# canyagmur/XPoint

Hardware: AMD Instinct MI355X
Metric: image-pairs/sec (detect+describe+match) 480x640 optical-thermal (higher is better)
Workload: dtype f32 (dense layers: f32 operands as 2 fp16 terms (operand error <= 2^-23, dropped cross term <= 2^-22: per product <= 2^-21 worst case, ~2^-25 typical), 3 fp16-MFMA partial products, f32 accumulate — GEMMs, implicit-GEMM convolutions and the fused block kernels alike; the deep-stage scan's dt project

## Files before the change

xpoint_amd/csrc/ss2d_chunked.hip:

```cpp
#include <string>

#include "ss2d_core.h"

namespace {

template <int R, typename UT = float>
__device__ __forceinline__ void stage_chunk(const SS2DParams& p, int T, int b, int pair, int chunk0, int* s_pix, int* s_off, float* s_x) {
    const int L = p.H * p.W;
    const int npx = p.cpb * T;
    const int tsh = 31 - __builtin_clz(T);
    for (int i = threadIdx.x; i < npx; i += blockDim.x) {
        int cl = i >> tsh, ii = i - (cl << tsh);
        int chunk = chunk0 + cl;
        const int px = (chunk < p.nc) ? pixel_of((chunk << tsh) + ii, L, p.H, p.W, pair == 1) : -1;
        s_pix[i] = px;
        s_off[i] = px >= 0 ? px * p.C : -1;
    }
    __syncthreads();
    constexpr int XW = 2 * (R + 2);
    constexpr int XD = 2 * XW;
    const UT* xsrc = reinterpret_cast<const UT*>(p.xdbl) + (int64_t)b * L * XD + pair * XW;
    for (int i = threadIdx.x; i < npx * XW; i += blockDim.x) {
        int pi = i / XW, e = i - pi * XW;
        int px = s_pix[pi];
        s_x[i] = (px >= 0) ? (float)xsrc[(int64_t)px * XD + e] : 0.f;
    }
    __syncthreads();
}

#define XP_PASS1_LOAD_U4(uv)                                                                                            \
    int px[4];                                                                                                          \
    _Pragma("unroll") for (int k = 0; k < 4; ++k) {                                                                     \
        px[k] = s_off[cl * p.T + i0 + k];                                                                               \
        const float t = (XP_SS2D_DBG & 8) ? 1.f : (float)ub[(FULL || px[k] >= 0) ? px[k] : 0];                          \
        uv[k] = (FULL || px[k] >= 0) ? t : 0.f;                                                                         \
    }

template <int R, bool FULL, bool AMP = false, typename UT = float>
__global__ __launch_bounds__(768) void ss2d_pass1(SS2DParams p) {
    constexpr float WL2E = AMP ? 1.f : XP_L2E;
    extern __shared__ __align__(16) char smem[];
    const int npx = p.cpb * p.T;
    int* s_pix = reinterpret_cast<int*>(smem);
    int* s_off = s_pix + npx;
    float* s_x = reinterpret_cast<float*>(smem + sizeof(int) * 2 * npx);
    constexpr int XW = 2 * (R + 2);
    const int b = blockIdx.y, pair = blockIdx.z, chunk0 = blockIdx.x * p.cpb;
    stage_chunk<R, UT>(p, p.T, b, pair, chunk0, s_pix, s_off, s_x);
    const int cl = threadIdx.x / p.C, c = threadIdx.x - cl * p.C;
    const int chunk = chunk0 + cl;
    if (chunk >= p.nc) return;
    const int L = p.H * p.W;
    const UT* ub = reinterpret_cast<const UT*>(p.u) + (int64_t)b * L * p.C + c;
    float P0 = 1.f, S0 = 0.f, Q1 = 1.f, S1 = 0.f;
    if constexpr (R < 16) {
        float w0[R], w1[R];
#pragma unroll
        for (int r = 0; r < R; ++r) {
            w0[r] = WL2E * p.wdt[((int64_t)(pair * 2 + 0) * R + r) * p.C + c];
            w1[r] = WL2E * p.wdt[((int64_t)(pair * 2 + 1) * R + r) * p.C + c];
        }
        const float b0 = WL2E * p.dtb[(pair * 2 + 0) * p.C + c], b1 = WL2E * p.dtb[(pair * 2 + 1) * p.C + c];
        const float A0 = XP_L2E * p.A[(pair * 2 + 0) * p.C + c], A1 = XP_L2E * p.A[(pair * 2 + 1) * p.C + c];
        for (int i0 = 0; i0 < p.T; i0 += 4) {
            float uv[4];
            XP_PASS1_LOAD_U4(uv)
#pragma unroll
            for (int k = 0; k < 4; ++k) {
                const float* xr = s_x + (cl * p.T + i0 + k) * XW;
                float a, bb, cv;
                step_vals<R, AMP>(xr, w0, b0, A0, uv[k], a, bb, cv);
                S0 = a * S0 + bb; P0 *= a;
                step_vals<R, AMP>(xr + (R + 2), w1, b1, A1, uv[k], a, bb, cv);
                S1 = fmaf(Q1, bb, S1); Q1 *= a;
            }
        }
    } else {
#pragma unroll 1
    for (int route = 0; route < 2; ++route) {
        float w[R];
#pragma unroll
        for (int r = 0; r < R; ++r) w[r] = WL2E * p.wdt[((int64_t)(pair * 2 + route) * R + r) * p.C + c];
        const float bias = WL2E * p.dtb[(pair * 2 + route) * p.C + c], Av = XP_L2E * p.A[(pair * 2 + route) * p.C + c];
        float Pr = 1.f, Sr = 0.f;
        for (int i0 = 0; i0 < p.T; i0 += 4) {
            float uv[4];
            XP_PASS1_LOAD_U4(uv)
#pragma unroll
            for (int k = 0; k < 4; ++k) {
                const float* xr = s_x + (cl * p.T + i0 + k) * XW + route * (R + 2);
                float a, bb, cv;
                step_vals<R, AMP>(xr, w, bias, Av, uv[k], a, bb, cv);
                if (route == 0) Sr = a * Sr + bb;
                else Sr = fmaf(Pr, bb, Sr);
                Pr *= a;
            }
        }
        if (route == 0) { P0 = Pr; S0 = Sr; } else { Q1 = Pr; S1 = Sr; }
    }
    }
    const int64_t o = ((((int64_t)b * 2 + pair) * p.nc + chunk) * 2) * p.C + c;
    p.wsP[o] = P0; p.wsS[o] = S0;
    p.wsP[o + p.C] = Q1; p.wsS[o + p.C] = S1;
}

#ifndef XP_SS2D_P2G
#define XP_SS2D_P2G 16
#endif
constexpr int P2_G = XP_SS2D_P2G;
__global__ __launch_bounds__(64 * P2_G) void ss2d_pass2(SS2DParams p) {
    __shared__ float s_P[P2_G][64], s_S[P2_G][64];
    const int lane = threadIdx.x, g = threadIdx.y;
    const int c = blockIdx.x * 64 + lane;
    const int bp = blockIdx.y >> 1, dir = blockIdx.y & 1;
    const bool ok = c < p.C;
    const int per = (p.nc + P2_G - 1) / P2_G;
    const int j0 = g * per, j1 = min(p.nc, j0 + per);
    auto off = [&](int jj) -> int64_t {
        const int j = dir ? (p.nc - 1 - jj) : jj;
        return (((int64_t)bp * p.nc + j) * 2 + dir) * p.C + c;
    };
    float P = 1.f, S = 0.f;
    if (ok) {
        int jj = j0;
        for (; jj + 4 <= j1; jj += 4) {
            float Pv[4], Sv[4];
#pragma unroll
            for (int k = 0; k < 4; ++k) { const int64_t o = off(jj + k); Pv[k] = p.wsP[o]; Sv[k] = p.wsS[o]; }
#pragma unroll
            for (int k = 0; k < 4; ++k) { S = fmaf(Pv[k], S, Sv[k]); P *= Pv[k]; }
        }
        for (; jj < j1; ++jj) { const int64_t o = off(jj); const float Pj = p.wsP[o], Sj = p.wsS[o]; S = fmaf(Pj, S, Sj); P *= Pj; }
    }
    s_P[g][lane] = P; s_S[g][lane] = S;
    __syncthreads();
    float h = 0.f;
    for (int gg = 0; gg < g; ++gg) h = fmaf(s_P[gg][lane], h, s_S[gg][lane]);
    if (!ok) return;
    int jj = j0;
    for (; jj + 4 <= j1; jj += 4) {
        float Pv[4], Sv[4];
        int64_t ov[4];
#pragma unroll
        for (int k = 0; k < 4; ++k) { ov[k] = off(jj + k); Pv[k] = p.wsP[ov[k]]; Sv[k] = p.wsS[ov[k]]; }
#pragma unroll
        for (int k = 0; k < 4; ++k) { p.wsS[ov[k]] = h; h = fmaf(Pv[k], h, Sv[k]); }
    }
    for (; jj < j1; ++jj) { const int64_t o = off(jj); const float Pj = p.wsP[o], Sj = p.wsS[o]; p.wsS[o] = h; h = fmaf(Pj, h, Sj); }
}

template <int R, bool COLPAIR, bool FULL, int T, bool AMP = false, typename UT = float>
__global__ __launch_bounds__(768) void ss2d_pass3(SS2DParams p) {
    constexpr float WL2E = AMP ? 1.f : XP_L2E;
    extern __shared__ __align__(16) char smem[];
    const int npx = p.cpb * T;
    int* s_pix = reinterpret_cast<int*>(smem);
    int* s_off = s_pix + npx;
    float* s_x = reinterpret_cast<float*>(smem + sizeof(int) * 2 * npx);
    constexpr int XW = 2 * (R + 2);
    float* s_y = s_x + npx * XW;
    const int SY = p.C + 8;
    const int pair = COLPAIR ? 1 : 0;
    const int b = blockIdx.y, chunk0 = blockIdx.x * p.cpb;
    stage_chunk<R, UT>(p, T, b, pair, chunk0, s_pix, s_off, s_x);
    const int cl = threadIdx.x / p.C, c = threadIdx.x - cl * p.C;
    const int chunk = chunk0 + cl;
    const int L = p.H * p.W;
    if (chunk < p.nc) {
        const int* so = s_off + cl * T;
        const float* sx = s_x + cl * T * XW;
        float* sy = s_y + cl * T * SY + c;
        const UT* ub = reinterpret_cast<const UT*>(p.u) + (int64_t)b * L * p.C + c;
        const float* prev = COLPAIR ? (p.ya + (int64_t)b * L * p.C + c) : nullptr;
        float* dst = COLPAIR ? nullptr : (p.ya + (int64_t)b * L * p.C + c);
        float w0[R];
#pragma unroll
        for (int r = 0; r < R; ++r) w0[r] = WL2E * p.wdt[((int64_t)(pair * 2 + 0) * R + r) * p.C + c];
        const float b0 = WL2E * p.dtb[(pair * 2 + 0) * p.C + c];
        const float A0 = XP_L2E * p.A[(pair * 2 + 0) * p.C + c];
        const float D0 = p.Dp[(pair * 2 + 0) * p.C + c];
        const int64_t o = ((((int64_t)b * 2 + pair) * p.nc + chunk) * 2) * p.C + c;
        float h = p.wsS[o];
        float uv[T], pv[COLPAIR ? T : 1];
#pragma unroll
        for (int i = 0; i < T; ++i) {
            const int off = so[i];
            const float t = (XP_SS2D_DBG & 8) ? 1.f : (float)ub[(FULL || off >= 0) ? off : 0];
            uv[i] = (FULL || off >= 0) ? t : 0.f;
            if ((i & 7) == 7) __builtin_amdgcn_sched_barrier(0);
        }
        if (COLPAIR) {
#pragma unroll
            for (int i = T - 1; i >= 0; --i) {
                const int off = so[i];
                pv[i] = (XP_SS2D_DBG & 2) ? 0.f : prev[(FULL || off >= 0) ? off : 0];
                if ((i & 7) == 0) __builtin_amdgcn_sched_barrier(0);
            }
        }
        __builtin_amdgcn_sched_barrier(0);
#pragma unroll
        for (int i0 = 0; i0 < T; i0 += 4) {
#pragma unroll
            for (int i = i0; i < i0 + 4; ++i) {
                float a, bb, cv;
                float ui = uv[i];
                asm("" : "+v"(ui));
                step_vals<R, AMP>(sx + i * XW, w0, b0, A0, ui, a, bb, cv);
                h = a * h + bb;
                sy[i * SY] = cv * h + D0 * ui;
            }
            __builtin_amdgcn_sched_barrier(0);
        }
        asm volatile("" ::: "memory");
        float w1[R];
#pragma unroll
        for (int r = 0; r < R; ++r) w1[r] = WL2E * p.wdt[((int64_t)(pair * 2 + 1) * R + r) * p.C + c];
        const float b1 = WL2E * p.dtb[(pair * 2 + 1) * p.C + c];
        const float A1 = XP_L2E * p.A[(pair * 2 + 1) * p.C + c];
        const float D1 = p.Dp[(pair * 2 + 1) * p.C + c];
        h = p.wsS[o + p.C];
        __builtin_amdgcn_sched_barrier(0);
#pragma unroll
        for (int i0 = T - 4; i0 >= 0; i0 -= 4) {
#pragma unroll
            for (int i = i0 + 3; i >= i0; --i) {
                float a, bb, cv;
                float ui = uv[i];
                asm("" : "+v"(ui));
                step_vals<R, AMP>(sx + i * XW + (R + 2), w1, b1, A1, ui, a, bb, cv);
                h = a * h + bb;
                const float y2 = cv * h + D1 * ui;
                float tot = sy[i * SY] + y2;
                if (COLPAIR) sy[i * SY] = pv[i] + tot;
                else {
                    asm volatile("" : "+v"(tot));
                    uv[i] = tot;
                }
            }
            __builtin_amdgcn_sched_barrier(0);
        }
        if (!COLPAIR) {
            asm volatile("" ::: "memory");
#pragma unroll
            for (int i = 0; i < T; ++i) {
                const int off = so[i];
                if (FULL || off >= 0) dst[off] = uv[i];
                if ((i & 7) == 7) __builtin_amdgcn_sched_barrier(0);
            }
        }
    }
    if (!COLPAIR) return;
    __syncthreads();
    if (XP_SS2D_DBG & 1) { if (threadIdx.x < 4) p.out[(int64_t)b * L * p.C + blockIdx.x * 4 + threadIdx.x] = s_y[threadIdx.x]; return; }
    const int wave = threadIdx.x >> 6, lane = threadIdx.x & 63, nw = blockDim.x >> 6;
    if (p.C <= 192) {
        const int sub = lane & 7, grp = lane >> 3;
        const int nj = p.C >> 5;
        const float invC = 1.f / (float)p.C;
        float4 gw[6], gb[6];
#pragma unroll
        for (int j = 0; j < 6; ++j)
            if (j < nj) {
                gw[j] = *reinterpret_cast<const float4*>(p.ln_w + 4 * (sub + 8 * j));
                gb[j] = *reinterpret_cast<const float4*>(p.ln_b + 4 * (sub + 8 * j));
            }
        for (int pi = wave * 8 + grp; pi < npx; pi += nw * 8) {
            const int px = s_pix[pi];
            if (px < 0) continue;
            const float* row = s_y + pi * SY;
            float4 r[6];
            float sm = 0.f;
#pragma unroll
            for (int j = 0; j < 6; ++j)
                if (j < nj) { r[j] = *reinterpret_cast<const float4*>(row + 4 * (sub + 8 * j)); sm += (r[j].x + r[j].y) + (r[j].z + r[j].w); }
            sm = xp_row8_sum(sm);
            const float mean = sm * invC;
            float v = 0.f;
#pragma unroll
            for (int j = 0; j < 6; ++j)
                if (j < nj) {
                    const float dx = r[j].x - mean, dy = r[j].y - mean, dz = r[j].z - mean, dw = r[j].w - mean;
                    v = fmaf(dx, dx, v); v = fmaf(dy, dy, v); v = fmaf(dz, dz, v); v = fmaf(dw, dw, v);
                }
            v = xp_row8_sum(v);
            const float rstd = 1.f / sqrtf(v * invC + p.eps);
            UT* orow = reinterpret_cast<UT*>(p.out) + ((int64_t)b * L + px) * p.C;
#pragma unroll
            for (int j = 0; j < 6; ++j)
                if (j < nj) {
                    float4 o;
                    o.x = (r[j].x - mean) * rstd * gw[j].x + gb[j].x; o.y = (r[j].y - mean) * rstd * gw[j].y + gb[j].y;
                    o.z = (r[j].z - mean) * rstd * gw[j].z + gb[j].z; o.w = (r[j].w - mean) * rstd * gw[j].w + gb[j].w;
                    if constexpr (std::is_same<UT, float>::value) *reinterpret_cast<float4*>(orow + 4 * (sub + 8 * j)) = o;
                    else {
                        union { _Float16 h[4]; uint2 u; } hh;
                        hh.h[0] = (_Float16)o.x; hh.h[1] = (_Float16)o.y; hh.h[2] = (_Float16)o.z; hh.h[3] = (_Float16)o.w;
                        *reinterpret_cast<uint2*>(orow + 4 * (sub + 8 * j)) = hh.u;
                    }
                }
        }
        return;
    }
    for (int pi = wave; pi < npx; pi += nw) {
        const int px = s_pix[pi];
        if (px < 0) continue;
        const float* row = s_y + pi * SY;
        float s = 0.f;
        for (int cc = lane; cc < p.C; cc += 64) s += row[cc];
        const float mean = xp_wave_sum(s) / (float)p.C;
        float v = 0.f;
        for (int cc = lane; cc < p.C; cc += 64) { float d = row[cc] - mean; v = fmaf(d, d, v); }
        const float rstd = 1.f / sqrtf(xp_wave_sum(v) / (float)p.C + p.eps);
        UT* orow = reinterpret_cast<UT*>(p.out) + ((int64_t)b * L + px) * p.C;
        for (int cc = lane; cc < p.C; cc += 64) orow[cc] = (UT)((row[cc] - mean) * rstd * p.ln_w[cc] + p.ln_b[cc]);
    }
}

typedef void (*ChunkKernel)(SS2DParams);
struct ChunkKernels {
    ChunkKernel pass1;
    ChunkKernel pass3[3][2];
};
template <int R, bool FULL, bool AMP, typename UT>
constexpr ChunkKernels chunk_kernels = {ss2d_pass1<R, FULL, AMP, UT>,
                                        {{ss2d_pass3<R, false, FULL, 8, AMP, UT>, ss2d_pass3<R, true, FULL, 8, AMP, UT>},
                                         {ss2d_pass3<R, false, FULL, 16, AMP, UT>, ss2d_pass3<R, true, FULL, 16, AMP, UT>},
                                         {ss2d_pass3<R, false, FULL, 32, AMP, UT>, ss2d_pass3<R, true, FULL, 32, AMP, UT>}}};
template <int R>
const ChunkKernels& chunk_class(bool half_io, bool amp, bool full) {
    static const ChunkKernels table[5] = {chunk_kernels<R, true, true, _Float16>, chunk_kernels<R, false, true, _Float16>, chunk_kernels<R, false, true, float>,
                                          chunk_kernels<R, true, false, float>, chunk_kernels<R, false, false, float>};
    return table[half_io ? (full ? 0 : 1) : (amp ? 2 : (full ? 3 : 4))];
}

template <int R>
int launch_ss2d(const SS2DParams& p, hipStream_t s, bool half_io) {
    constexpr int XW = 2 * (R + 2);
    const int npx = p.cpb * p.T;
    const int threads = p.cpb * p.C;
    const bool full = (p.H * p.W) % p.T == 0 && p.nc % p.cpb == 0;
    const ChunkKernels& k = chunk_class<R>(half_io, xp_amp_value() != 0, full);
    const int ti = p.T == 8 ? 0 : (p.T == 16 ? 1 : 2);
    const size_t sm1 = sizeof(int) * 2 * npx + sizeof(float) * npx * XW;
    const size_t sm3 = sm1 + sizeof(float) * (size_t)npx * (p.C + 8);
    dim3 grid1(xp_cdiv(p.nc, p.cpb), p.Bn, 2), grid3(xp_cdiv(p.nc, p.cpb), p.Bn, 1);
    const double MC = (double)p.Bn * p.H * p.W * p.C, MX = (double)p.Bn * p.H * p.W * XW;
    const std::string sfx = xp_prof_by_shape() ? "_C" + std::to_string(p.C) : std::string();
    const double el = 4.0 * MC;
    {
        XpProfScope prof(("ss2d_pass1" + sfx).c_str(), s, el * (2.0 * R + 12.0) / 2.0, 4.0 * 2.0 * (MC + MX));
        hipLaunchKernelGGL(k.pass1, grid1, dim3(threads), sm1, s, p);
    }
    {
        XpProfScope prof(("ss2d_pass2" + sfx).c_str(), s, 0.0, 4.0 * 3.0 * (double)p.Bn * 4 * p.nc * p.C);
        hipLaunchKernelGGL(ss2d_pass2, dim3(xp_cdiv(p.C, 64), p.Bn * 4), dim3(64, P2_G), 0, s, p);
    }
    {
        XpProfScope prof(("ss2d_pass3_row" + sfx).c_str(), s, el * (2.0 * R + 14.0) / 4.0, 4.0 * (2.0 * MC + MX));
        hipLaunchKernelGGL(k.pass3[ti][0], grid3, dim3(threads), sm3, s, p);
    }
    {
        XpProfScope prof(("ss2d_pass3_col_ln" + sfx).c_str(), s, el * (2.0 * R + 14.0) / 4.0, 4.0 * (3.0 * MC + MX));
        hipLaunchKernelGGL(k.pass3[ti][1], grid3, dim3(threads), sm3, s, p);
    }
    XP_LAUNCH_CHECK();
    return XP_OK;
}

}

int ss2d_launch_chunked(const SS2DParams& p, int R, bool half_io, hipStream_t s) {
    int rc = XP_ERR_ARG;
    SS2DRanks::dispatch(R, [&](auto r) { rc = launch_ss2d<decltype(r)::value>(p, s, half_io); });
    return rc;
}
```

xpoint_amd/csrc/ss2d_core.h:

```cpp
#pragma once
#include <type_traits>

#include "gemm_h2_core.h"
#include "xp_common.h"

#ifndef XP_SS2D_DBG
#define XP_SS2D_DBG 0
#endif

constexpr float XP_L2E =1.44269504088896340736f;

struct SS2DParams {
    const float* u;
    const float* xdbl;
    const float* wdt;
    const float* dtb;
    const float* A;
    const float* Dp;
    const float* ln_w;
    const float* ln_b;
    float* wsP;
    float* wsS;
    float* ya;
    float* out;
    int out_p32;
    int Bn, H, W, C, T, nc, cpb;
    float eps;
};

__device__ __forceinline__ int pixel_of(int l, int L, int H, int W, bool colmajor) {
    if (l >= L) return -1;
    if (!colmajor) return l;
    int w = l / H, h = l - w * H;
    return h * W + w;
}

template <int R, bool AMP = false>
__device__ __forceinline__ void step_vals(const float* __restrict__ xr, const float (&w)[R], float bias, float A,
                                          float u, float& a, float& b, float& Cv) {
    float xv[R + 2];
    if constexpr ((R + 2) % 4 == 0) {
#pragma unroll
        for (int q = 0; q < (R + 2) / 4; ++q) {
            const float4 t = *reinterpret_cast<const float4*>(xr + 4 * q);
            xv[4 * q] = t.x; xv[4 * q + 1] = t.y; xv[4 * q + 2] = t.z; xv[4 * q + 3] = t.w;
        }
    } else {
#pragma unroll
        for (int q = 0; q < (R + 2) / 2; ++q) {
            const float2 t = *reinterpret_cast<const float2*>(xr + 2 * q);
            xv[2 * q] = t.x; xv[2 * q + 1] = t.y;
        }
    }
    if (XP_SS2D_DBG & 4) { a = 0.5f; b = xv[R] * u; Cv = xv[R + 1]; return; }
    float dt;
    if constexpr (!AMP) {
        dt = fmaf(w[0], xv[0], bias);
#pragma unroll
        for (int r = 1; r < R; ++r) dt = fmaf(w[r], xv[r], dt);
    } else {
        dt = w[0] * xv[0];
#pragma unroll
        for (int r = 1; r < R; ++r) dt = fmaf(w[r], xv[r], dt);
        dt = ((float)(_Float16)dt + bias) * XP_L2E;
    }
    float delta;
    xp_softplus_decay_l2(dt, A, delta, a);
    b = delta * xv[R] * u;
    Cv = xv[R + 1];
}

template <int R>
struct DtWeights {
    static constexpr int KS = (R + 15) / 16;
    f16x8_t bw[2][KS][2];
    float bias[2];
    float bias_lane;
};
__device__ __forceinline__ void dt_split8(const float (&v)[8], f16x8_t& hi, f16x8_t& lo) {
    uint2 a0, a1, b0, b1;
    h2_split4(make_float4(v[0], v[1], v[2], v[3]), a0, a1);
    h2_split4(make_float4(v[4], v[5], v[6], v[7]), b0, b1);
    union { uint4 u; f16x8_t h; } x, y;
    x.u = make_uint4(a0.x, a0.y, b0.x, b0.y); y.u = make_uint4(a1.x, a1.y, b1.x, b1.y);
    hi = x.h; lo = y.h;
}
template <int R, bool AMP = false>
__device__ __forceinline__ void dt_load_weights(DtWeights<R>& w, const float* __restrict__ wdt_dir, const float* __restrict__ dtb_dir, int C, int cbase) {
    constexpr float WL2E = AMP ? 1.f : XP_L2E;
    const int fr = threadIdx.x & 31, fh = (threadIdx.x >> 5) & 1;
    w.bias_lane = dtb_dir[cbase + (threadIdx.x & 63)];
#pragma unroll
    for (int j = 0; j < 2; ++j) {
        const int cj = cbase + 32 * j + fr;
        w.bias[j] = AMP ? 0.f : XP_L2E * dtb_dir[cj];
#pragma unroll
        for (int ks = 0; ks < DtWeights<R>::KS; ++ks) {
            float wv[8];
#pragma unroll
            for (int e = 0; e < 8; ++e) {
                const int r = ks * 16 + fh * 8 + e;
                const float t = wdt_dir[(int64_t)(r < R ? r : 0) * C + cj];
                wv[e] = r < R ? WL2E * t : 0.f;
            }
            dt_split8(wv, w.bw[j][ks][0], w.bw[j][ks][1]);
        }
    }
}
template <int R, bool AMP = false>
__device__ __forceinline__ void dt_tile(const DtWeights<R>& w, const float* rows, int stride, float (&dtv)[2][16]) {
    const int fr = threadIdx.x & 31, fh = (threadIdx.x >> 5) & 1;
    f32x16 acc[2];
#pragma unroll
    for (int j = 0; j < 2; ++j) {
        float b0 = w.bias[j];
        if constexpr (!AMP) asm volatile("" : "+v"(b0));
#pragma unroll
        for (int e = 0; e < 16; ++e) acc[j][e] = b0;
    }
#pragma unroll
    for (int ks = 0; ks < DtWeights<R>::KS; ++ks) {
        const int k0 = ks * 16 + fh * 8;
        const float* ar = rows + fr * stride + (k0 < R ? k0 : 0);
        float v[8];
#pragma unroll
        for (int q = 0; q < 4; ++q) {
            const float2 t = *reinterpret_cast<const float2*>(ar + 2 * q);
            v[2 * q] = k0 + 2 * q < R ? t.x : 0.f;
            v[2 * q + 1] = k0 + 2 * q < R ? t.y : 0.f;
        }
        f16x8_t hi, lo;
        dt_split8(v, hi, lo);
#pragma unroll
        for (int j = 0; j < 2; ++j) {
            acc[j] = __builtin_amdgcn_mfma_f32_32x32x16_f16(lo, w.bw[j][ks][0], acc[j], 0, 0, 0);
            acc[j] = __builtin_amdgcn_mfma_f32_32x32x16_f16(hi, w.bw[j][ks][1], acc[j], 0, 0, 0);
            acc[j] = __builtin_amdgcn_mfma_f32_32x32x16_f16(hi, w.bw[j][ks][0], acc[j], 0, 0, 0);
        }
    }
#pragma unroll
    for (int e = 0; e < 16; ++e) {
        const auto sw = __builtin_amdgcn_permlane32_swap(__float_as_uint(acc[0][e]), __float_as_uint(acc[1][e]), false, false);
        dtv[0][e] = __uint_as_float(sw[0]); dtv[1][e] = __uint_as_float(sw[1]);
        if constexpr (AMP) {
            dtv[0][e] = ((float)(_Float16)dtv[0][e] + w.bias_lane) * XP_L2E;
            dtv[1][e] = ((float)(_Float16)dtv[1][e] + w.bias_lane) * XP_L2E;
        }
    }
}
#define XP_DTV(dtv, j) (dtv)[((j) >> 2) & 1][((j) & 3) + 4 * ((j) >> 3)]

template <int... Rs>
struct SS2DRankList {
    static bool has(int R) { return ((R == Rs) || ...); }
    template <typename F>
    static bool dispatch(int R, F&& f) { return ((R == Rs && (f(std::integral_constant<int, Rs>{}), true)) || ...); }
};
using SS2DRanks = SS2DRankList<2, 4, 6, 8, 12, 16, 24, 48>;

int ss2d_launch_chunked(const SS2DParams& p, int R, bool half_io, hipStream_t s);
int ss2d_launch_seq(const SS2DParams& p, float* ys, int R, bool half_out, hipStream_t s);
bool ss2d_seq_scan2_applies(int R, int H, int W, int C);
```

Before: 1835.

## Pad scan staging rows, prefetch u via buffer loads, and hold pass2 chunks in registers

```diff
diff --git a/xpoint_amd/csrc/ss2d_chunked.hip b/xpoint_amd/csrc/ss2d_chunked.hip
--- a/xpoint_amd/csrc/ss2d_chunked.hip
+++ b/xpoint_amd/csrc/ss2d_chunked.hip
@@ -4,6 +4,8 @@
 
 namespace {
 
+template <int R>
+constexpr int XRS = (R + 2 + 3) / 4 * 4;
 template <int R, typename UT = float>
 __device__ __forceinline__ void stage_chunk(const SS2DParams& p, int T, int b, int pair, int chunk0, int* s_pix, int* s_off, float* s_x) {
     const int L = p.H * p.W;
@@ -23,35 +25,62 @@
     for (int i = threadIdx.x; i < npx * XW; i += blockDim.x) {
         int pi = i / XW, e = i - pi * XW;
         int px = s_pix[pi];
-        s_x[i] = (px >= 0) ? (float)xsrc[(int64_t)px * XD + e] : 0.f;
+        const int at = (XRS<R> == R + 2) ? i : pi * (2 * XRS<R>) + e + (e >= R + 2 ? XRS<R> - (R + 2) : 0);
+        s_x[at] = (px >= 0) ? (float)xsrc[(int64_t)px * XD + e] : 0.f;
     }
     __syncthreads();
 }
 
-#define XP_PASS1_LOAD_U4(uv)                                                                                            \
-    int px[4];                                                                                                          \
-    _Pragma("unroll") for (int k = 0; k < 4; ++k) {                                                                     \
-        px[k] = s_off[cl * p.T + i0 + k];                                                                               \
-        const float t = (XP_SS2D_DBG & 8) ? 1.f : (float)ub[(FULL || px[k] >= 0) ? px[k] : 0];                          \
-        uv[k] = (FULL || px[k] >= 0) ? t : 0.f;                                                                         \
-    }
-
-template <int R, bool FULL, bool AMP = false, typename UT = float>
+constexpr uint32_t XP_SS2D_U_PAST = 0xFFFFFFF0u;
+template <typename UT>
+__device__ __forceinline__ float load_u32(__amdgpu_buffer_rsrc_t rs, int byte_off) {
+    if constexpr (std::is_same<UT, float>::value) return __builtin_bit_cast(float, __builtin_amdgcn_raw_buffer_load_b32(rs, byte_off, 0, 0));
+    else return (float)__builtin_bit_cast(_Float16, __builtin_amdgcn_raw_buffer_load_b16(rs, byte_off, 0, 0));
+}
+
+#ifndef XP_SS2D_P1_WIN
+#define XP_SS2D_P1_WIN 16
+#endif
+constexpr int P1_WIN = XP_SS2D_P1_WIN;
+
+template <int R, bool FULL, int T, bool AMP = false, typename UT = float>
 __global__ __launch_bounds__(768) void ss2d_pass1(SS2DParams p) {
     constexpr float WL2E = AMP ? 1.f : XP_L2E;
     extern __shared__ __align__(16) char smem[];
-    const int npx = p.cpb * p.T;
+    const int npx = p.cpb * T;
     int* s_pix = reinterpret_cast<int*>(smem);
     int* s_off = s_pix + npx;
     float* s_x = reinterpret_cast<float*>(smem + sizeof(int) * 2 * npx);
-    constexpr int XW = 2 * (R + 2);
+    constexpr int XS = 2 * XRS<R>;
     const int b = blockIdx.y, pair = blockIdx.z, chunk0 = blockIdx.x * p.cpb;
-    stage_chunk<R, UT>(p, p.T, b, pair, chunk0, s_pix, s_off, s_x);
+    stage_chunk<R, UT>(p, T, b, pair, chunk0, s_pix, s_off, s_x);
     const int cl = threadIdx.x / p.C, c = threadIdx.x - cl * p.C;
     const int chunk = chunk0 + cl;
     if (chunk >= p.nc) return;
     const int L = p.H * p.W;
-    const UT* ub = reinterpret_cast<const UT*>(p.u) + (int64_t)b * L * p.C + c;
+    const int* so = s_off + cl * T;
+    const float* sx = s_x + cl * T * XS;
+    const __amdgpu_buffer_rsrc_t ures = __builtin_amdgcn_make_buffer_rsrc(
+        const_cast<UT*>(reinterpret_cast<const UT*>(p.u) + (int64_t)b * L * p.C), 0, (int)((uint32_t)L * (uint32_t)p.C * (uint32_t)sizeof(UT)), 0x00020000);
+    const int cbytes = c * (int)sizeof(UT);
+    constexpr int USH = sizeof(UT) == 4 ? 2 : 1;
+    constexpr int UW = T < P1_WIN ? T : P1_WIN;
+    float uv[UW];
+#define XP_PASS1_LOAD_U(i)                                                                                                                     \
+    {                                                                                                                                          \
+        const int off = so[i];                                                                                                                 \
+        uv[(i) % UW] = (XP_SS2D_DBG & 8) ? 1.f : load_u32<UT>(ures, (FULL || off >= 0) ? (off << USH) + cbytes : (int)XP_SS2D_U_PAST);         \
+    }
+#define XP_PASS1_LOAD_FIRST                                           \
+    _Pragma("unroll") for (int i = 0; i < UW; ++i) {                  \
+        XP_PASS1_LOAD_U(i)                                            \
+        if ((i & 7) == 7) __builtin_amdgcn_sched_barrier(0);          \
+    }
+#define XP_PASS1_GROUP_END(i0, ...)                                                          \
+    asm volatile("" : __VA_ARGS__);                                                          \
+    if ((i0) + UW < T) { _Pragma("unroll") for (int k = 0; k < 4; ++k) XP_PASS1_LOAD_U((i0) + UW + k) } \
+    __builtin_amdgcn_sched_barrier(0);
+    XP_PASS1_LOAD_FIRST
     float P0 = 1.f, S0 = 0.f, Q1 = 1.f, S1 = 0.f;
     if constexpr (R < 16) {
         float w0[R], w1[R];
@@ -62,43 +91,61 @@
         }
         const float b0 = WL2E * p.dtb[(pair * 2 + 0) * p.C + c], b1 = WL2E * p.dtb[(pair * 2 + 1) * p.C + c];
         const float A0 = XP_L2E * p.A[(pair * 2 + 0) * p.C + c], A1 = XP_L2E * p.A[(pair * 2 + 1) * p.C + c];
-        for (int i0 = 0; i0 < p.T; i0 += 4) {
-            float uv[4];
-            XP_PASS1_LOAD_U4(uv)
-#pragma unroll
-            for (int k = 0; k < 4; ++k) {
-                const float* xr = s_x + (cl * p.T + i0 + k) * XW;
+        __builtin_amdgcn_sched_barrier(0);
+#pragma unroll
+        for (int i0 = 0; i0 < T; i0 += 4) {
+#pragma unroll
+            for (int i = i0; i < i0 + 4; ++i) {
+                const float* xr = sx + i * XS;
                 float a, bb, cv;
-                step_vals<R, AMP>(xr, w0, b0, A0, uv[k], a, bb, cv);
+                step_vals<R, AMP, true>(xr, w0, b0, A0, uv[i % UW], a, bb, cv);
                 S0 = a * S0 + bb; P0 *= a;
-                step_vals<R, AMP>(xr + (R + 2), w1, b1, A1, uv[k], a, bb, cv);
+                step_vals<R, AMP, true>(xr + XRS<R>, w1, b1, A1, uv[i % UW], a, bb, cv);
                 S1 = fmaf(Q1, bb, S1); Q1 *= a;
             }
+            XP_PASS1_GROUP_END(i0, "+v"(P0), "+v"(S0), "+v"(Q1), "+v"(S1))
         }
     } else {
-#pragma unroll 1
-    for (int route = 0; route < 2; ++route) {
-        float w[R];
-#pragma unroll
-        for (int r = 0; r < R; ++r) w[r] = WL2E * p.wdt[((int64_t)(pair * 2 + route) * R + r) * p.C + c];
-        const float bias = WL2E * p.dtb[(pair * 2 + route) * p.C + c], Av = XP_L2E * p.A[(pair * 2 + route) * p.C + c];
-        float Pr = 1.f, Sr = 0.f;
-        for (int i0 = 0; i0 < p.T; i0 += 4) {
-            float uv[4];
-            XP_PASS1_LOAD_U4(uv)
-#pragma unroll
-            for (int k = 0; k < 4; ++k) {
-                const float* xr = s_x + (cl * p.T + i0 + k) * XW + route * (R + 2);
-                float a, bb, cv;
-                step_vals<R, AMP>(xr, w, bias, Av, uv[k], a, bb, cv);
-                if (route == 0) Sr = a * Sr + bb;
-                else Sr = fmaf(Pr, bb, Sr);
-                Pr *= a;
-            }
-        }
-        if (route == 0) { P0 = Pr; S0 = Sr; } else { Q1 = Pr; S1 = Sr; }
-    }
-    }
+        {
+            float w[R];
+#pragma unroll
+            for (int r = 0; r < R; ++r) w[r] = WL2E * p.wdt[((int64_t)(pair * 2 + 0) * R + r) * p.C + c];
+            const float bias = WL2E * p.dtb[(pair * 2 + 0) * p.C + c], Av = XP_L2E * p.A[(pair * 2 + 0) * p.C + c];
+            __builtin_amdgcn_sched_barrier(0);
+#pragma unroll
+            for (int i0 = 0; i0 < T; i0 += 4) {
+#pragma unroll
+                for (int i = i0; i < i0 + 4; ++i) {
+                    float a, bb, cv;
+                    step_vals<R, AMP, true>(sx + i * XS, w, bias, Av, uv[i % UW], a, bb, cv);
+                    S0 = a * S0 + bb; P0 *= a;
+                }
+                XP_PASS1_GROUP_END(i0, "+v"(P0), "+v"(S0))
+            }
+        }
+        asm volatile("" ::: "memory");
+        {
+            if (T > UW) { XP_PASS1_LOAD_FIRST }
+            float w[R];
+#pragma unroll
+            for (int r = 0; r < R; ++r) w[r] = WL2E * p.wdt[((int64_t)(pair * 2 + 1) * R + r) * p.C + c];
+            const float bias = WL2E * p.dtb[(pair * 2 + 1) * p.C + c], Av = XP_L2E * p.A[(pair * 2 + 1) * p.C + c];
+            __builtin_amdgcn_sched_barrier(0);
+#pragma unroll
+            for (int i0 = 0; i0 < T; i0 += 4) {
+#pragma unroll
+                for (int i = i0; i < i0 + 4; ++i) {
+                    float a, bb, cv;
+                    step_vals<R, AMP, true>(sx + i * XS + XRS<R>, w, bias, Av, uv[i % UW], a, bb, cv);
+                    S1 = fmaf(Q1, bb, S1); Q1 *= a;
+                }
+                XP_PASS1_GROUP_END(i0, "+v"(Q1), "+v"(S1))
+            }
+        }
+    }
+#undef XP_PASS1_LOAD_U
+#undef XP_PASS1_LOAD_FIRST
+#undef XP_PASS1_GROUP_END
     const int64_t o = ((((int64_t)b * 2 + pair) * p.nc + chunk) * 2) * p.C + c;
     p.wsP[o] = P0; p.wsS[o] = S0;
     p.wsP[o + p.C] = Q1; p.wsS[o + p.C] = S1;
@@ -108,18 +155,60 @@
 #define XP_SS2D_P2G 16
 #endif
 constexpr int P2_G = XP_SS2D_P2G;
+constexpr int P2_HOLD = 40;
+template <int HOLD>
+__device__ __forceinline__ void pass2_held(const SS2DParams& p, float (*s_P)[64], float (*s_S)[64], int g, int lane, bool ok, int n, int64_t o0, int64_t step) {
+    float Pv[HOLD], Sv[HOLD];
+    const bool live = ok && n > 0;
+    if (live) {
+#pragma unroll
+        for (int k = 0; k < HOLD; ++k) {
+            const int64_t o = o0 + (k < n ? k : n - 1) * step;
+            Pv[k] = p.wsP[o]; Sv[k] = p.wsS[o];
+        }
+    }
+    float P = 1.f, S = 0.f;
+    if (live) {
+#pragma unroll
+        for (int k = 0; k < HOLD; ++k) {
+            const float Sn = fmaf(Pv[k], S, Sv[k]), Pn = P * Pv[k];
+            S = k < n ? Sn : S; P = k < n ? Pn : P;
+        }
+    }
+    s_P[g][lane] = P; s_S[g][lane] = S;
+    __syncthreads();
+    float h = 0.f;
+    for (int gg = 0; gg < g; ++gg) h = fmaf(s_P[gg][lane], h, s_S[gg][lane]);
+    if (!live) return;
+    float* dst = p.wsS + o0;
+#pragma unroll
+    for (int k = 0; k < HOLD; ++k)
+        if (k < n) { *dst = h; dst += step; h = fmaf(Pv[k], h, Sv[k]); }
+}
 __global__ __launch_bounds__(64 * P2_G) void ss2d_pass2(SS2DParams p) {
     __shared__ float s_P[P2_G][64], s_S[P2_G][64];
-    const int lane = threadIdx.x, g = threadIdx.y;
-    const int c = blockIdx.x * 64 + lane;
-    const int bp = blockIdx.y >> 1, dir = blockIdx.y & 1;
-    const bool ok = c < p.C;
+    const int lane = threadIdx.x;
+    const int g = __builtin_amdgcn_readfirstlane(threadIdx.y);
+    const int hpr = p.C >> 5;
+    const int hw = blockIdx.x * 2 + (lane >> 5);
+    const int row = hw / hpr;
+    const int c = (hw - row * hpr) * 32 + (lane & 31);
+    const int bp = row >> 1, dir = row & 1;
+    const bool ok = row < p.Bn * 4;
     const int per = (p.nc + P2_G - 1) / P2_G;
     const int j0 = g * per, j1 = min(p.nc, j0 + per);
     auto off = [&](int jj) -> int64_t {
         const int j = dir ? (p.nc - 1 - jj) : jj;
         return (((int64_t)bp * p.nc + j) * 2 + dir) * p.C + c;
     };
+    if (per <= P2_HOLD) {
+        const int n = j1 - j0;
+        const int64_t o0 = off(n > 0 ? j0 : 0), step = dir ? -2 * (int64_t)p.C : 2 * (int64_t)p.C;
+        if (per <= 8) pass2_held<8>(p, s_P, s_S, g, lane, ok, n, o0, step);
+        else if (per <= 24) pass2_held<24>(p, s_P, s_S, g, lane, ok, n, o0, step);
+        else pass2_held<P2_HOLD>(p, s_P, s_S, g, lane, ok, n, o0, step);
+        return;
+    }
     float P = 1.f, S = 0.f;
     if (ok) {
         int jj = j0;
@@ -157,7 +246,7 @@
     int* s_pix = reinterpret_cast<int*>(smem);
     int* s_off = s_pix + npx;
     float* s_x = reinterpret_cast<float*>(smem + sizeof(int) * 2 * npx);
-    constexpr int XW = 2 * (R + 2);
+    constexpr int XW = 2 * XRS<R>;
     float* s_y = s_x + npx * XW;
     const int SY = p.C + 8;
     const int pair = COLPAIR ? 1 : 0;
@@ -205,7 +294,7 @@
                 float a, bb, cv;
                 float ui = uv[i];
                 asm("" : "+v"(ui));
-                step_vals<R, AMP>(sx + i * XW, w0, b0, A0, ui, a, bb, cv);
+                step_vals<R, AMP, true>(sx + i * XW, w0, b0, A0, ui, a, bb, cv);
                 h = a * h + bb;
                 sy[i * SY] = cv * h + D0 * ui;
             }
@@ -227,7 +316,7 @@
                 float a, bb, cv;
                 float ui = uv[i];
                 asm("" : "+v"(ui));
-                step_vals<R, AMP>(sx + i * XW + (R + 2), w1, b1, A1, ui, a, bb, cv);
+                step_vals<R, AMP, true>(sx + i * XW + XRS<R>, w1, b1, A1, ui, a, bb, cv);
                 h = a * h + bb;
                 const float y2 = cv * h + D1 * ui;
                 float tot = sy[i * SY] + y2;
@@ -318,11 +407,11 @@
 
 typedef void (*ChunkKernel)(SS2DParams);
 struct ChunkKernels {
-    ChunkKernel pass1;
+    ChunkKernel pass1[3];
     ChunkKernel pass3[3][2];
 };
 template <int R, bool FULL, bool AMP, typename UT>
-constexpr ChunkKernels chunk_kernels = {ss2d_pass1<R, FULL, AMP, UT>,
+constexpr ChunkKernels chunk_kernels = {{ss2d_pass1<R, FULL, 8, AMP, UT>, ss2d_pass1<R, FULL, 16, AMP, UT>, ss2d_pass1<R, FULL, 32, AMP, UT>},
                                         {{ss2d_pass3<R, false, FULL, 8, AMP, UT>, ss2d_pass3<R, true, FULL, 8, AMP, UT>},
                                          {ss2d_pass3<R, false, FULL, 16, AMP, UT>, ss2d_pass3<R, true, FULL, 16, AMP, UT>},
                                          {ss2d_pass3<R, false, FULL, 32, AMP, UT>, ss2d_pass3<R, true, FULL, 32, AMP, UT>}}};
@@ -336,12 +425,13 @@
 template <int R>
 int launch_ss2d(const SS2DParams& p, hipStream_t s, bool half_io) {
     constexpr int XW = 2 * (R + 2);
+    XP_CHECK_ARG((int64_t)p.H * p.W * p.C * (half_io ? 2 : 4) < (int64_t)XP_SS2D_U_PAST, "xp_ss2d_core_fwd: one image plane (H*W*C) must stay below 2^32 - 16 bytes in the chunked form");
     const int npx = p.cpb * p.T;
     const int threads = p.cpb * p.C;
     const bool full = (p.H * p.W) % p.T == 0 && p.nc % p.cpb == 0;
     const ChunkKernels& k = chunk_class<R>(half_io, xp_amp_value() != 0, full);
     const int ti = p.T == 8 ? 0 : (p.T == 16 ? 1 : 2);
-    const size_t sm1 = sizeof(int) * 2 * npx + sizeof(float) * npx * XW;
+    const size_t sm1 = sizeof(int) * 2 * npx + sizeof(float) * npx * 2 * XRS<R>;
     const size_t sm3 = sm1 + sizeof(float) * (size_t)npx * (p.C + 8);
     dim3 grid1(xp_cdiv(p.nc, p.cpb), p.Bn, 2), grid3(xp_cdiv(p.nc, p.cpb), p.Bn, 1);
     const double MC = (double)p.Bn * p.H * p.W * p.C, MX = (double)p.Bn * p.H * p.W * XW;
@@ -349,11 +439,11 @@
     const double el = 4.0 * MC;
     {
         XpProfScope prof(("ss2d_pass1" + sfx).c_str(), s, el * (2.0 * R + 12.0) / 2.0, 4.0 * 2.0 * (MC + MX));
-        hipLaunchKernelGGL(k.pass1, grid1, dim3(threads), sm1, s, p);
+        hipLaunchKernelGGL(k.pass1[ti], grid1, dim3(threads), sm1, s, p);
     }
     {
         XpProfScope prof(("ss2d_pass2" + sfx).c_str(), s, 0.0, 4.0 * 3.0 * (double)p.Bn * 4 * p.nc * p.C);
-        hipLaunchKernelGGL(ss2d_pass2, dim3(xp_cdiv(p.C, 64), p.Bn * 4), dim3(64, P2_G), 0, s, p);
+        hipLaunchKernelGGL(ss2d_pass2, dim3(xp_cdiv(p.Bn * 4 * (p.C / 32), 2)), dim3(64, P2_G), 0, s, p);
     }
     {
         XpProfScope prof(("ss2d_pass3_row" + sfx).c_str(), s, el * (2.0 * R + 14.0) / 4.0, 4.0 * (2.0 * MC + MX));
diff --git a/xpoint_amd/csrc/ss2d_core.h b/xpoint_amd/csrc/ss2d_core.h
--- a/xpoint_amd/csrc/ss2d_core.h
+++ b/xpoint_amd/csrc/ss2d_core.h
@@ -35,13 +35,13 @@
     return h * W + w;
 }
 
-template <int R, bool AMP = false>
+template <int R, bool AMP = false, bool PAD4 = false>
 __device__ __forceinline__ void step_vals(const float* __restrict__ xr, const float (&w)[R], float bias, float A,
                                           float u, float& a, float& b, float& Cv) {
-    float xv[R + 2];
-    if constexpr ((R + 2) % 4 == 0) {
+    float xv[(R + 2 + 3) / 4 * 4];
+    if constexpr ((R + 2) % 4 == 0 || PAD4) {
 #pragma unroll
-        for (int q = 0; q < (R + 2) / 4; ++q) {
+        for (int q = 0; q < (R + 2 + 3) / 4; ++q) {
             const float4 t = *reinterpret_cast<const float4*>(xr + 4 * q);
             xv[4 * q] = t.x; xv[4 * q + 1] = t.y; xv[4 * q + 2] = t.z; xv[4 * q + 3] = t.w;
         }
```

Result: no change. 1842 (median of 2 runs) (+0.4%).
